# MingXiangL/SPE

Hardware: AMD Instinct MI355X
Metric: images/sec (whole node) at 3x800x1333 bs=2/GPU (higher is better)
Workload: dtype bf16/fp16 operands, fp32 accumulate; 1 GPU; TSCAM_cait_S24 (C=384, depth 24, 8 heads) + 0-layer encoder + 6-layer conditional-DETR decoder x2 stages, 100 queries, COCO heads (91), 2x3x800x1333 per GPU (N=4150 tokens), fwd + SetCriterion + SetCriterionRefine + bwd + grad all-reduce + clip + AdamW; global_batch=2, parallelism=dp1

## Files before the change

spe_amd/csrc/gemm_bf16tn.hip:

```cpp
#include "common.h"

#define GT_BR 64

typedef unsigned int u32x4t_t __attribute__((ext_vector_type(4)));
typedef short s16x4t_t __attribute__((ext_vector_type(4)));
typedef short s16x8t_t __attribute__((ext_vector_type(8)));

struct GemmTNArgs {
    const unsigned short* A; const unsigned short* B; float* C;
    int M, N, R; long lda, ldb, ldc; float alpha;
    int splitk; long slab; int rt_per_split;
};

template <int W>
__device__ __forceinline__ void gt_load(const unsigned short* __restrict__ base, long ld, int r0, int R, int c0, int C, u32x4t_t (&v)[W / 32]) {
    constexpr int CPR = W / 8, RPP = 256 / CPR;
    const int t = threadIdx.x, cc = c0 + (t % CPR) * 8;
    const bool cv = cc < C;
    const int ccl = cv ? cc : 0;
#pragma unroll
    for (int i = 0; i < W / 32; ++i) {
        const int r = r0 + t / CPR + RPP * i;
        const bool ok = cv && r < R;
        const u32x4t_t q = *reinterpret_cast<const u32x4t_t*>(base + (long)min(r, R - 1) * ld + ccl);
        v[i] = ok ? q : (u32x4t_t){0u, 0u, 0u, 0u};
    }
}
template <int W>
__device__ __forceinline__ void gt_stage(unsigned short* lds, const u32x4t_t (&v)[W / 32]) {
    constexpr int CPR = W / 8, RPP = 256 / CPR, LD = W + 8;
    const int t = threadIdx.x;
#pragma unroll
    for (int i = 0; i < W / 32; ++i)
        *reinterpret_cast<u32x4t_t*>(lds + (t / CPR + RPP * i) * LD + (t % CPR) * 8) = v[i];
}
template <int LD>
__device__ __forceinline__ bf16x8_t gt_operand(const unsigned short* tile, int ks, int c0, int lane) {
    typedef __attribute__((address_space(3))) s16x4t_t lds_s4;
    const unsigned short* p = tile + (32 * ks + 8 * (lane >> 4) + ((lane & 15) >> 2)) * LD + c0 + 4 * (lane & 3);
    const s16x4t_t v0 = __builtin_amdgcn_ds_read_tr16_b64_v4i16((lds_s4*)(p));
    const s16x4t_t v1 = __builtin_amdgcn_ds_read_tr16_b64_v4i16((lds_s4*)(p + 4 * LD));
    const s16x8t_t v = __builtin_shufflevector(v0, v1, 0, 1, 2, 3, 4, 5, 6, 7);
    return __builtin_bit_cast(bf16x8_t, v);
}

template <int BM, int BN>
__global__ __launch_bounds__(256) void gemm_bf16tn_kernel(GemmTNArgs p) {
    extern __shared__ __attribute__((aligned(16))) unsigned short smem_tn[];
    constexpr int NFM = BM / 32, NFN = BN / 32, WM = BM / 2, WN = BN / 2;
    constexpr int LDA = BM + 8, LDB = BN + 8;
    constexpr int TA_ = GT_BR * LDA, TB_ = GT_BR * LDB;
    auto sA = [&](int buf) { return smem_tn + buf * (TA_ + TB_); };
    auto sB = [&](int buf) { return smem_tn + buf * (TA_ + TB_) + TA_; };
    const int tiles_m = (p.M + BM - 1) / BM;
    const int tm = blockIdx.x % tiles_m, tn = blockIdx.x / tiles_m;
    const int zs = blockIdx.z;
    float* C = p.C + (long)zs * p.slab;
    const int m0 = tm * BM, n0 = tn * BN;
    const int rtiles = (p.R + GT_BR - 1) / GT_BR;
    const int rt_begin = zs * p.rt_per_split;
    int rt_end = rt_begin + p.rt_per_split; if (rt_end > rtiles) rt_end = rtiles;
    const int nt = rt_end - rt_begin;
    const int lane = threadIdx.x & 63, w = threadIdx.x >> 6;
    const int wm = w >> 1, wn = w & 1, fr = lane & 15;

    f32x4_t acc[NFM][NFN];
#pragma unroll
    for (int i = 0; i < NFM; ++i)
#pragma unroll
        for (int j = 0; j < NFN; ++j) acc[i][j] = (f32x4_t){0.f, 0.f, 0.f, 0.f};

    u32x4t_t ca[BM / 32], cb[BN / 32], na[BM / 32], nb[BN / 32];
#pragma unroll
    for (int i = 0; i < BM / 32; ++i) na[i] = (u32x4t_t){0u, 0u, 0u, 0u};
#pragma unroll
    for (int i = 0; i < BN / 32; ++i) nb[i] = (u32x4t_t){0u, 0u, 0u, 0u};
    if (nt > 0) {
        gt_load<BM>(p.A, p.lda, rt_begin * GT_BR, p.R, m0, p.M, ca);
        gt_load<BN>(p.B, p.ldb, rt_begin * GT_BR, p.R, n0, p.N, cb);
        gt_stage<BM>(sA(0), ca);
        gt_stage<BN>(sB(0), cb);
        if (nt > 1) {
            gt_load<BM>(p.A, p.lda, (rt_begin + 1) * GT_BR, p.R, m0, p.M, ca);
            gt_load<BN>(p.B, p.ldb, (rt_begin + 1) * GT_BR, p.R, n0, p.N, cb);
        }
        __syncthreads();
        for (int t = 0; t < nt; ++t) {
            const int buf = t & 1;
            if (t + 2 < nt) {
                gt_load<BM>(p.A, p.lda, (rt_begin + t + 2) * GT_BR, p.R, m0, p.M, na);
                gt_load<BN>(p.B, p.ldb, (rt_begin + t + 2) * GT_BR, p.R, n0, p.N, nb);
            }
#pragma unroll
            for (int ks = 0; ks < GT_BR / 32; ++ks) {
                bf16x8_t a[NFM], b[NFN];
#pragma unroll
                for (int i = 0; i < NFM; ++i) a[i] = gt_operand<LDA>(sA(buf), ks, wm * WM + i * 16, lane);
#pragma unroll
                for (int j = 0; j < NFN; ++j) b[j] = gt_operand<LDB>(sB(buf), ks, wn * WN + j * 16, lane);
#pragma unroll
                for (int i = 0; i < NFM; ++i)
#pragma unroll
                    for (int j = 0; j < NFN; ++j)
                        acc[i][j] = __builtin_amdgcn_mfma_f32_16x16x32_bf16(b[j], a[i], acc[i][j], 0, 0, 0);
            }
            if (t + 1 < nt) {
                gt_stage<BM>(sA(buf ^ 1), ca);
                gt_stage<BN>(sB(buf ^ 1), cb);
            }
#pragma unroll
            for (int i = 0; i < BM / 32; ++i) ca[i] = na[i];
#pragma unroll
            for (int i = 0; i < BN / 32; ++i) cb[i] = nb[i];
            __syncthreads();
        }
    }
    const bool vst = ((p.ldc & 3) == 0) && ((reinterpret_cast<uintptr_t>(C) & 15) == 0);
#pragma unroll
    for (int j = 0; j < NFN; ++j) {
        const int n = n0 + wn * WN + j * 16 + (lane >> 4) * 4;
        if (n >= p.N) continue;
#pragma unroll
        for (int i = 0; i < NFM; ++i) {
            const int m = m0 + wm * WM + i * 16 + fr;
            if (m >= p.M) continue;
            const long off = (long)m * p.ldc + n;
            float v[4];
#pragma unroll
            for (int r = 0; r < 4; ++r) v[r] = acc[i][j][r] * p.alpha;
            if (vst && n + 3 < p.N) spe_store4_stream(C + off, v[0], v[1], v[2], v[3]);
            else {
#pragma unroll
                for (int r = 0; r < 4; ++r) if (n + r < p.N) C[off + r] = v[r];
            }
        }
    }
}

template <int BM, int BN>
static int launch_tn(const GemmTNArgs& p, hipStream_t stream) {
    constexpr int smem = 2 * GT_BR * ((BM + 8) + (BN + 8)) * (int)sizeof(unsigned short);
    static bool attr_set = false;
    if (!attr_set) {
        hipError_t e = hipFuncSetAttribute(reinterpret_cast<const void*>(&gemm_bf16tn_kernel<BM, BN>),
                                           hipFuncAttributeMaxDynamicSharedMemorySize, smem);
        if (e != hipSuccess) return (int)e;
        attr_set = true;
    }
    const int tiles = ((p.M + BM - 1) / BM) * ((p.N + BN - 1) / BN);
    hipLaunchKernelGGL((gemm_bf16tn_kernel<BM, BN>), dim3(tiles, 1, p.splitk), dim3(256), smem, stream, p);
    SPE_CHECK_LAUNCH();
    return 0;
}

extern "C" int spe_gemm_bf16tn(const void* A16, const void* B16, float* C, int M, int N, int R, long lda, long ldb, long ldc,
                               float alpha, int splitk, hipStream_t stream) {
    if (M <= 0 || N <= 0) return 0;
    if (R <= 0) return -4;
    auto al16 = [](const void* q) { return (reinterpret_cast<uintptr_t>(q) & 15) == 0; };
    if (!al16(A16) || !al16(B16) || (lda & 7) || (ldb & 7) || (M & 7) || (N & 7)) return -2;
    GemmTNArgs p;
    p.A = reinterpret_cast<const unsigned short*>(A16); p.B = reinterpret_cast<const unsigned short*>(B16); p.C = C;
    p.M = M; p.N = N; p.R = R; p.lda = lda; p.ldb = ldb; p.ldc = ldc; p.alpha = alpha; p.slab = 0;
    const int rtiles = (R + GT_BR - 1) / GT_BR;
    if (splitk < 0) { splitk = -splitk; p.slab = (long)M * ldc; if (splitk > rtiles) return -5; }
    else if (splitk > 1) return -2;
    if (splitk < 1) splitk = 1;
    p.splitk = splitk;
    p.rt_per_split = (rtiles + splitk - 1) / splitk;
    const long t128 = (long)((M + 127) / 128) * ((N + 127) / 128) * splitk;
    static const int small_max = SPE_KNOB("SPE_TN_SMALL_TILES", 256);
    if (t128 < small_max) return launch_tn<64, 64>(p, stream);
    if (M > 64 && N > 64) return launch_tn<128, 128>(p, stream);
    if (M > 64) return launch_tn<128, 64>(p, stream);
    return launch_tn<64, 64>(p, stream);
}
```

spe_amd/kernels.py:

```python
import ctypes
import os

import torch

from . import lib

_PRECISION = 2
import functools as _functools
import threading as _threading

_TLS = _threading.local()


def _in_bwd():
    return getattr(_TLS, "in_bwd", False)


def backward_scope(fn):
    @_functools.wraps(fn)
    def wrapped(ctx, *grads):
        prev, _TLS.in_bwd = _in_bwd(), True
        if _DEFER_FLATS is not None and not _FLUSH_QUEUED[0]:
            _FLUSH_QUEUED[0] = True
            try:
                torch.autograd.Variable._execution_engine.queue_callback(_flush_after_backward)
            except RuntimeError:
                _FLUSH_QUEUED[0] = False
        try:
            return fn(ctx, *grads)
        finally:
            _TLS.in_bwd = prev
    return wrapped


_FLUSH_QUEUED = [False]
_DEFER_FLATS = None


def _flush_after_backward():
    _FLUSH_QUEUED[0] = False
    reduce_flush()


def forward_scope(fn):
    @_functools.wraps(fn)
    def wrapped(ctx, *args):
        prev, _TLS.in_bwd = _in_bwd(), False
        try:
            return fn(ctx, *args)
        finally:
            _TLS.in_bwd = prev
    return wrapped


def split_now():
    return _PRECISION == 1 or (_PRECISION == 2 and not _in_bwd())


def split_fwd():
    return _PRECISION == 2 and not _in_bwd()
_RNG = {"seed": None, "offset": 0}


def set_precision(mode):
    global _PRECISION
    _PRECISION = {"bf16": 0, "bf16x3": 1, "bf16s": 2, 0: 0, 1: 1, 2: 2}[mode]


def get_precision():
    return ("bf16", "bf16x3", "bf16s")[_PRECISION]


def manual_seed(seed):
    _RNG["seed"] = int(seed) & 0xFFFFFFFFFFFFFFFF
    _RNG["offset"] = 0


def next_rng():
    if _RNG["seed"] is None:
        _RNG["seed"] = (torch.initial_seed() * 0x9E3779B97F4A7C15 + 0x5EEDC0DE) & 0xFFFFFFFFFFFFFFFF
    _RNG["offset"] += 1
    return _RNG["seed"], _RNG["offset"]


_TIMED = {}


def enable_timing(names):
    _TIMED.clear()
    for n in names:
        _TIMED[n] = []


def timing_results():
    return {n: (len(ev), (sum(a.elapsed_time(b) for a, b in ev) / len(ev)) if ev else 0.0) for n, ev in _TIMED.items()}


_GEMM_DIMS = {"spe_gemm_bf16nt": (7, 8, 9), "spe_gemm_bf16nt_ex": (16, 17, 18)}


_RWS = None
_RWS_BYTES = 16 << 20


_RWS_DEVIDX = -1
_RWS_STREAM = None


def _register_reduce_ws():
    global _RWS
    dev = torch.device("cuda", torch.cuda.current_device())
    _RWS = torch.zeros((_RWS_BYTES,), device=dev, dtype=torch.uint8)
    lib.call("spe_set_reduce_workspace", _RWS.data_ptr(), _RWS_BYTES, _st())


def _guard_reduce_ws(cur, st):
    global _RWS_STREAM, _RWS_DEVIDX
    if _RWS is None:
        _register_reduce_ws()
    if cur != _RWS.device.index:
        raise lib.SpeLibraryError(f"spe_amd kernels were first used on cuda:{_RWS.device.index} and are now launched on cuda:{cur}: "
                                  "the reduction workspace is per process (one process per GPU)")
    if _RWS_STREAM is not None and st != _RWS_STREAM:
        ev = torch.cuda.Event()
        ev.record(torch.cuda.ExternalStream(_RWS_STREAM, device=_RWS.device) if _RWS_STREAM else torch.cuda.default_stream(_RWS.device))
        torch.cuda.current_stream().wait_event(ev)
    _RWS_STREAM, _RWS_DEVIDX = st, cur


DEFER_REDUCE = os.environ.get("SPE_DEFER_REDUCE", "1") != "0"
_DEFER_ARENA = None


def defer_reductions(flats, arena_bytes=48 << 20):
    global _DEFER_ARENA, _DEFER_FLATS
    if _DEFER_FLATS is not None:
        lib.call("spe_reduce_flush", _st())
    if not flats or not DEFER_REDUCE or not flats[0].is_cuda or flats[0].dtype != torch.float32:
        lib.call("spe_reduce_defer_ranges", None, None, 0)
        _DEFER_FLATS = None
        return
    if _DEFER_ARENA is None or _DEFER_ARENA.device != flats[0].device:
        _DEFER_ARENA = torch.empty((arena_bytes,), device=flats[0].device, dtype=torch.uint8)
        lib.call("spe_reduce_defer_arena", _DEFER_ARENA.data_ptr(), arena_bytes)
    n = len(flats)
    ptrs = (ctypes.c_void_p * n)(*[f.data_ptr() for f in flats])
    sizes = (ctypes.c_size_t * n)(*[f.numel() * 4 for f in flats])
    lib.call("spe_reduce_defer_ranges", ptrs, sizes, n)
    _DEFER_FLATS = list(flats)


def reduce_flush():
    if _DEFER_FLATS is not None:
        lib.call("spe_reduce_flush", _st())


def _call(name, *args):
    if _RWS is None:
        _register_reduce_ws()
    if not _TIMED:
        return lib.call(name, *args)
    ev = _TIMED.get(name)
    if ev is None and name in _GEMM_DIMS:
        i, j, k = _GEMM_DIMS[name]
        ev = _TIMED.get("%s:%d,%d,%d" % (name, args[i], args[j], args[k]))
    if ev is None:
        return lib.call(name, *args)
    a, b = torch.cuda.Event(enable_timing=True), torch.cuda.Event(enable_timing=True)
    a.record()
    lib.call(name, *args)
    b.record()
    ev.append((a, b))


_ZPOOL = {"buf": None, "off": 0}
_ZPOOL_FLOATS = 4 << 20


def zeros_small(n, device):
    if n > (1 << 18):
        return torch.zeros((n,), device=device, dtype=torch.float32)
    na = (n + 63) & ~63
    z = _ZPOOL
    if z["buf"] is None or z["buf"].device != device or z["off"] + na > z["buf"].numel():
        z["buf"] = torch.zeros((_ZPOOL_FLOATS,), device=device, dtype=torch.float32)
        z["off"] = 0
    out = z["buf"][z["off"]:z["off"] + n]
    z["off"] += na
    return out


def grad_buffer(param):
    if param is None or not getattr(param, "_spe_grad_fresh", False) or getattr(param, "_spe_shared", False):
        return None
    param._spe_grad_fresh = False
    param._spe_handed = True
    buf = param._spe_grad_buf
    return buf.view_as(buf)


ACC_ZERO_MAX = 16384


def _zeros_or(buf, n, device):
    if buf is None:
        return zeros_small(n, device)
    v = buf.view(-1)
    if v.numel() > ACC_ZERO_MAX:
        v.zero_()
    return v


def _p(t):
    return None if t is None else t.data_ptr()


_raw_stream = getattr(torch._C, "_cuda_getCurrentRawStream", None)


def _st():
    cur = torch.cuda.current_device()
    st = _raw_stream(cur) if _raw_stream is not None else torch.cuda.current_stream().cuda_stream
    if st != _RWS_STREAM or cur != _RWS_DEVIDX:
        _guard_reduce_ws(cur, st)
    return st


def _chk(*ts):
    for t in ts:
        if t is None:
            continue
        if not t.is_cuda:
            raise lib.SpeLibraryError("spe_amd kernels run on the GPU only (got a CPU tensor); there is no CPU fallback")
        if t.dtype != torch.float32:
            raise TypeError(f"expected float32, got {t.dtype}")


TN_SMALL_MAX = 256


def auto_splitk(M, N, K, batch):
    tiles = ((M + 127) // 128) * ((N + 127) // 128) * batch
    if tiles >= 256 or K < 1024:
        return 1
    sk = max(1, min(512 // tiles, K // 512, 16))
    if batch == 1 and tiles * sk < TN_SMALL_MAX:
        t64 = ((M + 63) // 64) * ((N + 63) // 64)
        sk = max(1, min(512 // t64, K // 512, 16))
    return sk


def gemm(A, B, C, M, N, K, lda, ldb, ldc, transA=False, transB=False, bias=None, C2=None,
         batch0=1, batch1=1, sA=(0, 0), sB=(0, 0), sC=(0, 0), alpha=1.0, act=0, splitk=1):
    _call("spe_gemm_f32", _p(A), _p(B), _p(C), _p(bias), _p(C2), M, N, K, lda, ldb, ldc,
             int(transA), int(transB), batch0, batch1, sA[0], sA[1], sB[0], sB[1], sC[0], sC[1],
             float(alpha), int(act), int(splitk), int(split_now()), _st())
    return C


LINEAR16 = True
LINEAR16_MIN_ROWS = 128
_W16 = {}
_W16_EPOCH = 0


def weights_changed():
    global _W16_EPOCH
    _W16_EPOCH += 1


LINEAR_SMALL_MAX_ROWS = 2048


def _lin_small_ok(R, N, K):
    return LINEAR16 and _PRECISION != 1 and LINEAR16_MIN_ROWS <= R < LINEAR_SMALL_MAX_ROWS and N % 8 == 0 and K % 8 == 0


def _lin16_ok(R, N, K):
    return LINEAR16 and _PRECISION != 1 and R >= LINEAR16_MIN_ROWS and N % 8 == 0 and K % 8 == 0


def cvt_bf16(x2, want=True, wantT=False, ldt=None, colsum_out=None, act_aux=None, act=0, out=None, ldo=None, out_lo=None, lo_f16=False):
    _chk(x2)
    R, C = x2.shape
    if out is None:
        out = torch.empty((R, C), device=x2.device, dtype=torch.bfloat16) if want else None
        ldo = C
    outT = None
    if wantT:
        ldt = ldt or ((R + 63) // 64) * 64
        outT = torch.empty((C, ldt), device=x2.device, dtype=torch.bfloat16)
    if lo_f16:
        assert colsum_out is None and act_aux is None and out_lo is not None and out_lo.dtype == torch.float16
        _call("spe_cvt_bf16_h", _p(x2), x2.stride(0), R, C, _p(out), _p(out_lo), ldo or C, _p(outT), ldt or 0, _st())
        return out, outT
    _call("spe_cvt_bf16", _p(x2), x2.stride(0), R, C, _p(out), _p(out_lo), ldo or C, _p(outT), ldt or 0, _p(colsum_out), _p(act_aux),
          int(act), _st())
    return out, outT


_W16_TABLE = None
_W16_REFRESHED = -1


def _refresh_weights16():
    global _W16_TABLE, _W16_REFRESHED
    import numpy as np
    live = []
    for key, ent in list(_W16.items()):
        owner = ent[0]()
        if owner is None or not _owns(owner, key[0]):
            del _W16[key]
            continue
        live.append((key, owner, ent))
    _W16_REFRESHED = _W16_EPOCH
    if not live:
        return
    sig = tuple((k, e[3].data_ptr(), e[4].data_ptr(), e[5].data_ptr() if e[5] is not None else 0, e[5].dtype if e[5] is not None else None)
                for k, _, e in live)
    if _W16_TABLE is None or _W16_TABLE[0] != sig:
        rec = np.zeros(len(live), dtype=np.dtype([("x", "<u8"), ("out", "<u8"), ("outT", "<u8"), ("ldt", "<i8"), ("R", "<i4"),
                                                   ("C", "<i4"), ("tile0", "<i4"), ("tiles_c", "<i4"), ("out_lo", "<u8"), ("flags", "<i8")]))
        t0 = 0
        for i, ((ptr, R, C), _, e) in enumerate(live):
            tc = (C + 63) // 64
            rec[i] = (ptr, e[3].data_ptr(), e[4].data_ptr(), e[4].shape[1], R, C, t0, tc, e[5].data_ptr() if e[5] is not None else 0,
                      1 if (e[5] is not None and e[5].dtype == torch.float16) else 0)
            t0 += tc * ((max(R, e[4].shape[1]) + 63) // 64)
        table = host_table(rec.view(np.uint8), live[0][2][3].device)
        _W16_TABLE = (sig, table, len(live), t0)
    _, table, n, tiles = _W16_TABLE
    _call("spe_cvt_bf16_multi", _p(table), n, tiles, _st())
    for key, owner, e in live:
        _W16[key] = (e[0], owner._version, _W16_EPOCH, e[3], e[4], e[5])


def _owns(owner, ptr):
    base = owner.data_ptr()
    return base <= ptr < base + max(1, owner.numel()) * owner.element_size()


def host_table(bytes_np, device):
    pin = torch.from_numpy(bytes_np.copy()).pin_memory()
    dev = torch.empty(pin.shape, dtype=torch.uint8, device=device)
    dev.copy_(pin, non_blocking=True)
    dev._spe_pin = pin
    return dev


def weight16(W, lo=False, f16=False):
    import weakref
    key = (W.data_ptr(), W.shape[0], W.shape[1])
    ent = _W16.get(key)
    if ent is not None:
        owner = ent[0]()
        if owner is not None and _owns(owner, key[0]):
            if ent[2] != _W16_EPOCH and _W16_REFRESHED != _W16_EPOCH:
                _refresh_weights16()
                ent = _W16.get(key, ent)
            if ent[1] == owner._version and ent[2] == _W16_EPOCH and (not lo or (ent[5] is not None and (ent[5].dtype == torch.float16) == f16)):
                return (ent[3], ent[4], ent[5]) if lo else (ent[3], ent[4])
            if not lo and ent[5] is not None and ent[5].dtype == torch.float16:
                f16 = True
    owner = W._base if W._base is not None else W
    want_lo = lo or f16 or _PRECISION == 2
    with torch.no_grad():
        W16lo = torch.empty(W.shape, device=W.device, dtype=torch.float16 if f16 else torch.bfloat16) if want_lo else None
        W16, W16T = cvt_bf16(W.detach(), True, True, ldt=W.shape[0], out_lo=W16lo, lo_f16=f16)
    if len(_W16) > 4096:
        _W16.clear()
    _W16[key] = (weakref.ref(owner), owner._version, _W16_EPOCH, W16, W16T, W16lo)
    return (W16, W16T, W16lo) if lo else (W16, W16T)


_WCAT = {}


def weightcat16(Ws, bs, lo=False):
    import weakref
    key = tuple((W.data_ptr(), tuple(W.shape)) for W in Ws)
    vers = tuple(W._version for W in Ws) + tuple(b._version for b in bs)
    ent = _WCAT.get(key)
    if ent is not None and ent[1] == _W16_EPOCH and ent[2] == vers and (ent[6] is not None or not lo):
        owners = [r() for r in ent[0]]
        if all(o is not None and _owns(o, W.data_ptr()) for o, W in zip(owners, Ws)) and ent[3].shape == (sum(W.shape[0] for W in Ws), Ws[0].shape[1]):
            return (ent[3], ent[4], ent[5], ent[6]) if lo else (ent[3], ent[4], ent[5])
    with torch.no_grad():
        trip = [weight16(W, lo=lo) for W in Ws]
        Wc = torch.cat([t_[0] for t_ in trip], 0)
        WcT = torch.cat([t_[1] for t_ in trip], 1)
        Wclo = torch.cat([t_[2] for t_ in trip], 0) if lo else None
        bc = torch.cat([b.detach() for b in bs])
    if len(_WCAT) > 64:
        _WCAT.clear()
    _WCAT[key] = ([weakref.ref(W._base if W._base is not None else W) for W in Ws], _W16_EPOCH, vers, Wc, WcT, bc, Wclo)
    return (Wc, WcT, bc, Wclo) if lo else (Wc, WcT, bc)


def gemm_splitk_into(A, B, out, M, N, K, lda, ldb, ldc, transA, transB, batch0, batch1, sA, sB, sC, alpha=1.0):
    sk = auto_splitk(M, N, K, batch0 * batch1)
    if sk <= 1:
        return gemm(A, B, out, M, N, K, lda, ldb, ldc, transA, transB, batch0=batch0, batch1=batch1, sA=sA, sB=sB, sC=sC, alpha=alpha)
    extent = (((batch0 - 1) * sC[0] + (batch1 - 1) * sC[1] + (M - 1) * ldc + N) + 3) & ~3
    assert out.is_contiguous() and extent <= out.numel() + 3
    ws = torch.empty((sk, extent), device=out.device, dtype=torch.float32)
    gemm(A, B, ws, M, N, K, lda, ldb, ldc, transA, transB, batch0=batch0, batch1=batch1, sA=sA, sB=sB, sC=sC, alpha=alpha, splitk=-sk)
    out.zero_()
    n = out.numel()
    _call("spe_colsum", _p(ws), _p(out), sk, n, extent, 1, _st())
    return out


def gemm16(A16, B16, C, M, N, K, lda, ldb, ldc, bias=None, C2=None, alpha=1.0, act=0, splitk=1, Alo=None, Blo=None):
    _call("spe_gemm_bf16nt", _p(A16), _p(B16), _p(Alo), _p(Blo), _p(C), _p(bias), _p(C2), M, N, K, lda, ldb, ldc, float(alpha), int(act),
          int(splitk), _st())
    return C


def cvt_f16(x2, out=None):
    R, C = x2.shape
    if out is None:
        out = torch.empty((R, C), device=x2.device, dtype=torch.float16)
    _call("spe_cvt_f16", _p(x2), x2.stride(0), R, C, _p(out), out.stride(0), _st())
    return out


_WCATH = {}


def weightcat_f16(Ws, bs):
    import weakref
    key = tuple((W.data_ptr(), tuple(W.shape)) for W in Ws)
    vers = tuple(W._version for W in Ws) + tuple(b._version for b in bs)
    ent = _WCATH.get(key)
    if ent is not None and ent[1] == _W16_EPOCH and ent[2] == vers:
        owners = [r() for r in ent[0]]
        if all(o is not None and _owns(o, W.data_ptr()) for o, W in zip(owners, Ws)):
            return ent[3], ent[4]
    with torch.no_grad():
        Wh = cvt_f16(torch.cat([W.detach() for W in Ws], 0))
        bc = torch.cat([b.detach() for b in bs])
    if len(_WCATH) > 64:
        _WCATH.clear()
    _WCATH[key] = ([weakref.ref(W._base if W._base is not None else W) for W in Ws], _W16_EPOCH, vers, Wh, bc)
    return Wh, bc


def kv_frags(ym16, yp16, L, B, S, H, dh, train):
    dev = ym16.device
    nt, dk = (S + 15) // 16, 2 * dh
    Kf = torch.empty((L, B, H, nt, (dk + 31) // 32, 64, 8), device=dev, dtype=torch.float16)
    V16 = torch.empty((L, B, H, nt, (dh + 15) // 16, 64, 4), device=dev, dtype=torch.float16)
    K16 = torch.empty((L, B, H, nt, (dk + 15) // 16, 64, 4), device=dev, dtype=torch.bfloat16) if train else None
    Vf = torch.empty((L, B, H, nt, (dh + 31) // 32, 64, 8), device=dev, dtype=torch.bfloat16) if train else None
    _call("spe_kv_frags", _p(ym16), ym16.stride(0), _p(yp16), yp16.stride(0), _p(Kf), _p(V16), _p(K16), _p(Vf), L, B, S, H, dh, _st())
    return Kf, V16, K16, Vf


def kv_grad_scatter(dk, dv, dYm, dYp, layer, B, S, H, dh):
    _call("spe_kv_grad_scatter", _p(dk), _p(dv), _p(dYm), dYm.stride(0), _p(dYp), dYp.stride(0), int(layer), B, S, H, dh, _st())


def colsum_bf16_blocks(x16, blkC, outs):
    n = len(outs)
    ptrs = (ctypes.c_void_p * n)(*[o.data_ptr() for o in outs])
    _call("spe_colsum_bf16_blocks", _p(x16), x16.stride(0), x16.shape[0], n, int(blkC), ptrs, 0, _st())


def gemm16_tn(A16, B16, C, M, N, R, lda, ldb, ldc, alpha=1.0, splitk=1):
    _call("spe_gemm_bf16tn", _p(A16), _p(B16), _p(C), M, N, R, lda, ldb, ldc, float(alpha), int(splitk), _st())
    return C


def gemm16_ex(A16, B16, M, N, K, lda, ldb, bias=None, C=None, C2=None, out16=None, out16T=None, colsum=None, aux=None,
              alpha=1.0, act=0, res=None, rgamma=None, Alo=None, Blo=None, out16lo=None, drop=None, sscale=None, rps=1, op_f16=False):
    half_flags = (1 if (C2 is not None and C2.dtype == torch.float16) else 0) | (2 if (aux is not None and aux.dtype == torch.float16) else 0)
    if op_f16:
        assert A16.dtype == torch.float16 and B16.dtype == torch.float16 and Alo is None and Blo is None
        half_flags |= 4 | (8 if out16lo is not None else 0)
        assert out16lo is None or out16lo.dtype == torch.float16
    if (drop is not None and drop[0] > 0) or sscale is not None:
        pd, sd, of = drop if (drop is not None and drop[0] > 0) else (0.0, 0, 0)
        _call("spe_gemm_bf16nt_exd", _p(A16), _p(B16), _p(Alo), _p(Blo), _p(C), _p(bias), _p(C2), _p(out16), _p(out16lo), N, _p(out16T),
              out16T.shape[1] if out16T is not None else 0, _p(colsum), _p(aux), _p(res), _p(rgamma), M, N, K, lda, ldb, N,
              float(alpha), int(act), half_flags, float(pd), int(sd), int(of), _p(sscale), int(rps), _st())
        return
    _call("spe_gemm_bf16nt_ex", _p(A16), _p(B16), _p(Alo), _p(Blo), _p(C), _p(bias), _p(C2), _p(out16), _p(out16lo), N, _p(out16T),
          out16T.shape[1] if out16T is not None else 0, _p(colsum), _p(aux), _p(res), _p(rgamma), M, N, K, lda, ldb, N,
          float(alpha), int(act), half_flags, _st())


def mlp16_ok(R, K, Hd, N):
    return _lin16_ok(R, Hd, K) and _lin16_ok(R, N, Hd)




def layerscale_residual_bwd16(dout2, y2, gamma, Rp, db_out=None, dg_out=None, want_rowmajor=True, want_T=True, drop=None, sscale=None, rps=1):
    R, C = dout2.shape
    dev = dout2.device
    dy16 = torch.empty((R, C), device=dev, dtype=torch.bfloat16) if want_rowmajor else None
    dy16T = torch.empty((C, Rp), device=dev, dtype=torch.bfloat16) if want_T else None
    db = _zeros_or(db_out, C, dev)
    dg = _zeros_or(dg_out, C, dev)
    if (drop is not None and drop[0] > 0) or sscale is not None:
        pd, sd, of = drop if (drop is not None and drop[0] > 0) else (0.0, 0, 0)
        _call("spe_layerscale_residual_bwd16d", _p(dout2), _p(y2), int(y2.dtype == torch.float16), _p(gamma), _p(dy16), _p(dy16T), Rp, _p(db),
              _p(dg), R, C, float(pd), int(sd), int(of), _p(sscale), int(rps), _st())
        return dy16, dy16T, db, dg
    _call("spe_layerscale_residual_bwd16", _p(dout2), _p(y2), int(y2.dtype == torch.float16), _p(gamma), _p(dy16), _p(dy16T), Rp, _p(db), _p(dg),
          R, C, _st())
    return dy16, dy16T, db, dg


def linear_res_fwd(x2, W, b, res, gamma, save=True, src=None, drop=None, sscale=None, rps=1):
    R, K = x2.shape
    N = W.shape[0]
    dev = x2.device
    sp = split_fwd()
    x16, x16lo = act16(x2, src, want_lo=sp)
    out = torch.empty((R, N), device=dev, dtype=torch.float32)
    y = torch.empty((R, N), device=dev, dtype=torch.float16 if MLP_PRE_F16 else torch.float32) if save else None
    Wt = weight16(W, lo=sp)
    gemm16_ex(x16, Wt[0], R, N, K, K, K, bias=b, C=out, C2=y, res=res, rgamma=gamma, Alo=x16lo, Blo=Wt[2] if sp else None,
              drop=drop, sscale=sscale, rps=rps)
    return out, (x16, y)


def linear_res_bwd(dout2, saved, W, gamma, need_dx=True, grad_bufs=(None, None, None), drop=None, sscale=None, rps=1, pre=None):
    x16, y = saved
    R, N = dout2.shape
    K = W.shape[1]
    gW, gb, gg = grad_bufs
    if pre is not None:
        dy16, db, dg = pre
    else:
        dy16, _, db, dg = layerscale_residual_bwd16(dout2, y, gamma, ((R + 63) // 64) * 64, db_out=gb, dg_out=gg, want_rowmajor=True, want_T=False,
                                                    drop=drop, sscale=sscale, rps=rps)
    dW = _dw16_tn(dy16, x16, N, K, R, gW)
    dx = None
    if need_dx:
        dx = torch.empty((R, K), device=dout2.device, dtype=torch.float32)
        gemm16(dy16, weight16(W)[1], dx, R, K, N, N, N, K)
    return dx, dW, db, dg


MLP_PRE_F16 = False


MLP_F16 = True


def mlp_f16_ok(R, K, Hd, N):
    return (MLP_F16 and split_fwd() and R >= 2048 and K % 64 == 0 and K >= 128 and Hd % 64 == 0 and Hd >= 128 and N % 8 == 0 and N >= 64)


def mlp_gelu_fwd(x2, W1, b1, W2, b2, res=None, gamma=None, save=True, src=None, drop1=None, drop2=None, sscale=None, rps=1):
    R, K = x2.shape
    Hd, N = W1.shape[0], W2.shape[0]
    dev = x2.device
    sp = split_fwd()
    if res is not None and mlp_f16_ok(R, K, Hd, N):
        x16, xh = act16(x2, src, want_lo=True, lo_f16=True)
        pre = torch.empty((R, Hd), device=dev, dtype=torch.float16 if MLP_PRE_F16 else torch.float32) if save else None
        h16 = torch.empty((R, Hd), device=dev, dtype=torch.bfloat16)
        hh = torch.empty((R, Hd), device=dev, dtype=torch.float16)
        W1h, W2h = weight16(W1, lo=True, f16=True)[2], weight16(W2, lo=True, f16=True)[2]
        gemm16_ex(xh, W1h, R, Hd, K, K, K, bias=b1, C2=pre, out16=h16, act=2, out16lo=hh, drop=drop1, op_f16=True)
        out = torch.empty((R, N), device=dev, dtype=torch.float32)
        y = torch.empty((R, N), device=dev, dtype=torch.float16 if MLP_PRE_F16 else torch.float32) if save else None
        gemm16_ex(hh, W2h, R, N, Hd, Hd, Hd, bias=b2, C=out, C2=y, res=res, rgamma=gamma, drop=drop2, sscale=sscale, rps=rps, op_f16=True)
        return out, (x16, pre, h16, y)
    x16, x16lo = act16(x2, src, want_lo=sp)
    pre = torch.empty((R, Hd), device=dev, dtype=torch.float16 if MLP_PRE_F16 else torch.float32) if save else None
    h16 = torch.empty((R, Hd), device=dev, dtype=torch.bfloat16)
    h16lo = torch.empty((R, Hd), device=dev, dtype=torch.bfloat16) if sp else None
    W1t, W2t = weight16(W1, lo=sp), weight16(W2, lo=sp)
    W1lo, W2lo = (W1t[2], W2t[2]) if sp else (None, None)
    gemm16_ex(x16, W1t[0], R, Hd, K, K, K, bias=b1, C2=pre, out16=h16, act=2, Alo=x16lo, Blo=W1lo, out16lo=h16lo, drop=drop1)
    y = torch.empty((R, N), device=dev, dtype=torch.float32)
    if res is None:
        gemm16(h16, W2t[0], y, R, N, Hd, Hd, Hd, N, bias=b2, Alo=h16lo, Blo=W2lo)
        return y, (x16, pre, h16)
    out = torch.empty((R, N), device=dev, dtype=torch.float32)
    if MLP_PRE_F16:
        y = torch.empty((R, N), device=dev, dtype=torch.float16)
    gemm16_ex(h16, W2t[0], R, N, Hd, Hd, Hd, bias=b2, C=out, C2=y if save else None, res=res, rgamma=gamma, Alo=h16lo, Blo=W2lo,
              drop=drop2, sscale=sscale, rps=rps)
    return out, (x16, pre, h16, y)


def _dw_slabs(launch, sk, N, K, dW_out, dev):
    if sk > 1:
        ws = torch.empty((sk, N * K), device=dev, dtype=torch.float32)
        launch(ws, -sk)
        return colsum(ws, out=None if dW_out is None else dW_out.view(-1), accumulate=dW_out is None).view(N, K)
    dW = dW_out if dW_out is not None else torch.empty((N, K), device=dev, dtype=torch.float32)
    launch(dW, 1)
    return dW


def _dw16_tn(dy16, x16, N, K, R, dW_out, lda=None):
    lda = N if lda is None else lda
    sk = min(auto_splitk(N, K, R, 1), max(1, R // 64))
    return _dw_slabs(lambda C, splitk: gemm16_tn(dy16, x16, C, N, K, R, lda, K, K, splitk=splitk), sk, N, K, dW_out, dy16.device)


def mlp_gelu_bwd(dy2, saved, W1, W2, need_dx=True, grad_bufs=(None, None, None, None), gamma=None, dg_out=None,
                 drop1=None, drop2=None, sscale=None, rps=1, ls_pre=None):
    x16, pre, h16 = saved[:3]
    R, N = dy2.shape
    Hd, K = W1.shape
    dev = dy2.device
    gW1, gb1, gW2, gb2 = grad_bufs
    dg = None
    if ls_pre is not None and gamma is None:
        raise RuntimeError("spe_amd.kernels.mlp_gelu_bwd: a LayerNorm backward took this node's LayerScale part, but the node cannot consume it")
    if ls_pre is not None:
        dy16, db2, dg = ls_pre
    elif gamma is not None:
        dy16, _, db2, dg = layerscale_residual_bwd16(dy2, saved[3], gamma, ((R + 63) // 64) * 64, db_out=gb2, dg_out=dg_out, want_T=False,
                                                     drop=drop2, sscale=sscale, rps=rps)
    else:
        db2 = _zeros_or(gb2, N, dev)
        dy16, _ = cvt_bf16(dy2, True, False, colsum_out=db2)
    dW2 = _dw16_tn(dy16, h16, N, Hd, R, gW2)
    db1 = _zeros_or(gb1, Hd, dev)
    dp16 = torch.empty((R, Hd), device=dev, dtype=torch.bfloat16)
    gemm16_ex(dy16, weight16(W2)[1], R, Hd, N, N, N, out16=dp16, colsum=db1, aux=pre, act=2, drop=drop1)
    dW1 = _dw16_tn(dp16, x16, Hd, K, R, gW1)
    dx = None
    if need_dx:
        dx = torch.empty((R, K), device=dev, dtype=torch.float32)
        gemm16(dp16, weight16(W1)[1], dx, R, K, Hd, Hd, Hd, K)
    if gamma is not None:
        return dx, dW1, db1, dW2, db2, dg
    return dx, dW1, db1, dW2, db2


def act16(x2, src=None, want_lo=False, lo_f16=False):
    if src is not None:
        ent = getattr(src, "_spe16", None)
        if (ent is not None and ent[0] == src._version and ent[1].shape == x2.shape
                and (not want_lo or (ent[3] is not None and (ent[3].dtype == torch.float16) == lo_f16))):
            return ent[1], (ent[3] if want_lo else None)
    x16lo = torch.empty(x2.shape, device=x2.device, dtype=torch.float16 if lo_f16 else torch.bfloat16) if want_lo else None
    x16, _ = cvt_bf16(x2, True, False, out_lo=x16lo, lo_f16=lo_f16 and want_lo)
    if src is not None:
        attach16(src, x16, x16lo)
    return x16, x16lo


def linear_fwd(x2, W, b, act=0, want_pre=False, save_for_dw=True, src=None):
    _chk(x2, W, b)
    R, K = x2.shape
    N = W.shape[0]
    y = torch.empty((R, N), device=x2.device, dtype=torch.float32)
    pre = torch.empty_like(y) if want_pre else None
    if _lin_small_ok(R, N, K) and W.is_contiguous():
        sp = split_fwd()
        Wt = weight16(W, lo=sp)
        ent = getattr(src, "_spe16", None) if src is not None else None
        x16 = ent[1] if (ent is not None and ent[0] == src._version and ent[1].shape == x2.shape) else None
        x16_out = None
        if x16 is None and save_for_dw:
            x16 = x16_out = torch.empty((R, K), device=x2.device, dtype=torch.bfloat16)
            if src is not None:
                attach16(src, x16)
        _call("spe_linear_small_fwd", _p(x2), x2.stride(0), _p(Wt[0]), _p(Wt[2] if sp else None), _p(b), _p(y), _p(pre), _p(x16_out),
              R, N, K, N, int(act), _st())
        return y, pre, (x16 if save_for_dw else x2)
    if _lin16_ok(R, N, K) and W.is_contiguous():
        sp = split_fwd()
        x16, x16lo = act16(x2, src, want_lo=sp)
        Wt = weight16(W, lo=sp)
        gemm16(x16, Wt[0], y, R, N, K, K, K, N, bias=b, C2=pre, act=act, Alo=x16lo, Blo=Wt[2] if sp else None)
        return y, pre, (x16 if save_for_dw else x2)
    gemm(x2, W, y, R, N, K, K, K, N, False, True, bias=b, C2=pre, act=act)
    return y, pre, x2


def linear_group_ok(R, Ws, bs):
    N, K = Ws[0].shape
    return (2 <= len(Ws) <= 16 and _lin_small_ok(R, N, K) and N % 128 == 0
            and all(W.shape == Ws[0].shape and W.is_contiguous() for W in Ws) and all(b is not None for b in bs))


def _ptr_array(ptrs):
    return (ctypes.c_void_p * len(ptrs))(*[(p if p else None) for p in ptrs])


def linear_group_fwd(x2, Ws, bs, src=None, adds=None):
    _chk(x2, *Ws)
    R, K = x2.shape
    N = Ws[0].shape[0]
    sp = split_fwd()
    trip = [weight16(W, lo=sp) for W in Ws]
    ent = getattr(src, "_spe16", None) if src is not None else None
    x16 = ent[1] if (ent is not None and ent[0] == src._version and ent[1].shape == x2.shape) else None
    x16_out = None
    if x16 is None:
        x16 = x16_out = torch.empty((R, K), device=x2.device, dtype=torch.bfloat16)
        if src is not None:
            attach16(src, x16)
    ys = [torch.empty((R, N), device=x2.device, dtype=torch.float32) for _ in Ws]
    _call("spe_linear_small_group_fwd", _p(x2), x2.stride(0), _ptr_array([t_[0].data_ptr() for t_ in trip]),
          _ptr_array([t_[2].data_ptr() for t_ in trip]) if sp else None, _ptr_array([b.data_ptr() for b in bs]),
          _ptr_array([0 if a is None else a.data_ptr() for a in adds]) if adds is not None else None,
          _ptr_array([y.data_ptr() for y in ys]), _p(x16_out), R, len(Ws), N, K, _st())
    return ys, x16


def linear_group_bwd(dys, x16, Ws, need_dx, dW_outs, db_outs):
    n = len(Ws)
    N, K = Ws[0].shape
    R = x16.shape[0]
    dev = x16.device
    dx = torch.empty((R, K), device=dev, dtype=torch.float32) if need_dx else None
    dWs, dbs = [], []
    for i in range(n):
        if dys[i] is None:
            dWs.append(None); dbs.append(None)
            continue
        dWs.append(dW_outs[i] if dW_outs[i] is not None else torch.empty((N, K), device=dev, dtype=torch.float32))
        dbs.append(db_outs[i].view(-1) if db_outs[i] is not None else torch.empty((N,), device=dev, dtype=torch.float32))
    _call("spe_linear_small_group_bwd", _ptr_array([0 if d is None else d.data_ptr() for d in dys]), _p(x16),
          _ptr_array([weight16(W)[1].data_ptr() for W in Ws]) if need_dx else None, _p(dx),
          _ptr_array([0 if w is None else w.data_ptr() for w in dWs]), _ptr_array([0 if b is None else b.data_ptr() for b in dbs]),
          R, n, N, K, _st())
    return dx, dWs, dbs


def linear_bwd(dy2, xsave, W, need_dx=True, need_dw=True, need_db=True, dW_out=None, db_out=None, act=0, act_aux=None):
    _chk(dy2, W)
    R, N = dy2.shape
    K = W.shape[1]
    dx = dW = db = None
    x16 = xsave.dtype == torch.bfloat16
    if (x16 or not need_dw) and _lin_small_ok(R, N, K) and W.is_contiguous():
        dev = dy2.device
        if need_dx:
            dx = torch.empty((R, K), device=dev, dtype=torch.float32)
        if need_dw:
            dW = dW_out if dW_out is not None else torch.empty((N, K), device=dev, dtype=torch.float32)
        if need_db:
            db = db_out.view(-1) if db_out is not None else torch.empty((N,), device=dev, dtype=torch.float32)
        _call("spe_linear_small_bwd", _p(dy2), _p(act_aux if act else None), int(act), _p(xsave if need_dw else None),
              _p(weight16(W)[1] if need_dx else None), _p(dx), _p(dW), _p(db), R, N, K, _st())
        return dx, dW, db
    if (x16 or not need_dw) and _lin16_ok(R, N, K) and W.is_contiguous():
        if need_db:
            db = _zeros_or(db_out, N, dy2.device)
        dy16, _ = cvt_bf16(dy2, need_dx or need_dw, False, colsum_out=db, act_aux=act_aux if act else None, act=act)
        need_db = False
        if need_dx:
            dx = torch.empty((R, K), device=dy2.device, dtype=torch.float32)
            gemm16(dy16, weight16(W)[1], dx, R, K, N, N, N, K)
        if need_dw:
            dW = _dw16_tn(dy16, xsave, N, K, R, dW_out)
    else:
        if x16:
            raise RuntimeError("linear_bwd: bf16 activations were saved but the bf16 GEMM path is disabled now")
        if act:
            dy2 = act_bwd(dy2, act_aux, act)
        x2 = xsave
        if need_dx:
            dx = torch.empty((R, K), device=dy2.device, dtype=torch.float32)
            gemm(dy2, W, dx, R, K, N, N, K, K, False, False)
        if need_dw:
            dW = _dw_slabs(lambda C, splitk: gemm(dy2, x2, C, N, K, R, N, K, K, True, False, splitk=splitk), auto_splitk(N, K, R, 1), N, K,
                           dW_out, dy2.device)
    if need_db:
        db = _zeros_or(db_out, N, dy2.device)
        _call("spe_colsum", _p(dy2), _p(db), R, N, N, 1, _st())
    return dx, dW, db


def colsum(x2, out=None, accumulate=True):
    _chk(x2)
    R, C = x2.shape
    if out is None:
        out = zeros_small(C, x2.device)
    _call("spe_colsum", _p(x2), _p(out), R, C, x2.stride(0), int(bool(accumulate)), _st())
    return out


def act_bwd(dy, aux, mode):
    _chk(dy, aux)
    dx = torch.empty_like(dy)
    _call("spe_act_bwd", _p(dy), _p(aux), _p(dx), dy.numel(), mode, _st())
    return dx


def layernorm_fwd(x2, g, b, eps, want16=False, f16=False):
    _chk(x2, g, b)
    R, C = x2.shape
    y = torch.empty_like(x2)
    mean = torch.empty((R,), device=x2.device, dtype=torch.float32)
    rstd = torch.empty_like(mean)
    y16 = torch.empty((R, C), device=x2.device, dtype=torch.bfloat16) if want16 else None
    f16 = f16 and want16 and split_fwd()
    y16lo = torch.empty((R, C), device=x2.device, dtype=torch.float16 if f16 else torch.bfloat16) if (want16 and split_fwd()) else None
    _call("spe_layernorm_fwd_h" if f16 else "spe_layernorm_fwd", _p(x2), _p(g), _p(b), _p(y), _p(mean), _p(rstd), R, C, float(eps), _p(y16), _p(y16lo), _st())
    return (y, mean, rstd, y16, y16lo) if want16 else (y, mean, rstd)


def produces16(R, C):
    return LINEAR16 and _PRECISION != 1 and R >= LINEAR16_MIN_ROWS and C % 8 == 0


def attach16(t, x16, x16lo=None):
    t._spe16 = (t._version, x16, None, x16lo)


LN_LS_FUSE = True


def layernorm_bwd(dy2, x2, g, mean, rstd, dg_out=None, db_out=None, add=None, ls=None):
    _chk(dy2, x2, g)
    R, C = x2.shape
    dx = torch.empty_like(x2)
    dg = _zeros_or(dg_out, C, x2.device)
    db = _zeros_or(db_out, C, x2.device)
    if ls is not None:
        y, lgam, ls_db_out, ls_dg_out = ls
        dy16 = torch.empty((R, C), device=x2.device, dtype=torch.bfloat16)
        ldb = _zeros_or(ls_db_out, C, x2.device)
        ldg = _zeros_or(ls_dg_out, C, x2.device)
        _call("spe_layernorm_bwd_ls", _p(dy2), _p(x2), _p(g), _p(mean), _p(rstd), _p(dx), _p(dg), _p(db), R, C, _p(add), _p(y), _p(lgam), _p(dy16),
              _p(ldb), _p(ldg), _st())
        return dx, dg, db, (dy16, ldb, ldg)
    _call("spe_layernorm_bwd", _p(dy2), _p(x2), _p(g), _p(mean), _p(rstd), _p(dx), _p(dg), _p(db), R, C, _p(add), _st())
    return dx, dg, db


def layernorm_res_fwd(x2, z2, g, b, eps, p, seed, offset):
    _chk(x2, z2, g, b)
    R, C = x2.shape
    y, sm = torch.empty_like(x2), torch.empty_like(x2)
    mean = torch.empty((R,), device=x2.device, dtype=torch.float32)
    rstd = torch.empty_like(mean)
    _call("spe_layernorm_res_fwd", _p(x2), _p(z2), _p(g), _p(b), _p(sm), _p(y), _p(mean), _p(rstd), R, C, float(eps), float(p), seed,
          offset, _st())
    return y, sm, mean, rstd


def layernorm_res_bwd(dy2, sm, g, mean, rstd, p, seed, offset, dg_out=None, db_out=None, dy_b=None):
    R, C = sm.shape
    ds = torch.empty_like(sm)
    dz = torch.empty_like(sm) if p > 0 else None
    dg = _zeros_or(dg_out, C, sm.device)
    db = _zeros_or(db_out, C, sm.device)
    _call("spe_layernorm_res_bwd", _p(dy2), _p(dy_b), _p(sm), _p(g), _p(mean), _p(rstd), _p(ds), _p(dz), _p(dg), _p(db), R, C, float(p), seed,
          offset, _st())
    return ds, (dz if dz is not None else ds), dg, db


def layerscale_residual_fwd(x2, y2, gamma, sample_scale, rows_per_sample):
    _chk(x2, y2, gamma, sample_scale)
    R, C = x2.shape
    out = torch.empty_like(x2)
    _call("spe_layerscale_residual_fwd", _p(x2), _p(y2), _p(gamma), _p(sample_scale), _p(out), R, C,
             rows_per_sample, _st())
    return out


def layerscale_residual_bwd(dout2, y2, gamma, sample_scale, rows_per_sample, dg_out=None):
    _chk(dout2, y2, gamma, sample_scale)
    R, C = dout2.shape
    dy = torch.empty_like(dout2)
    dg = _zeros_or(dg_out, C, dout2.device)
    _call("spe_layerscale_residual_bwd", _p(dout2), _p(y2), _p(gamma), _p(sample_scale), _p(dy), _p(dg), R, C,
             rows_per_sample, _st())
    return dy, dg


def dropout(x, p, seed, offset):
    _chk(x)
    y = torch.empty_like(x)
    _call("spe_dropout", _p(x), _p(y), x.numel(), float(p), seed, offset, _st())
    return y


def pad4(n):
    return (n + 3) // 4 * 4


def softmax_fwd(S, mask_u8, B, H, Nq, Nk, ld, p_drop, seed, offset):
    Pd = torch.empty_like(S) if p_drop > 0 else None
    _call("spe_softmax_fwd", _p(S), _p(mask_u8), _p(S), _p(Pd), B, H, Nq, Nk, ld, float(p_drop), seed, offset, _st())
    return S, Pd


def softmax_bwd(dPd, P, B, H, Nq, Nk, ld, p_drop, seed, offset):
    _call("spe_softmax_bwd", _p(dPd), _p(P), _p(dPd), B, H, Nq, Nk, ld, float(p_drop), seed, offset, _st())
    return dPd


def talking_fwd(S, Wl, bl, Ww, bw, B, H, Nq, Nk, ld, p_drop, seed, offset):
    Pd = torch.empty_like(S)
    _call("spe_talking_softmax_fwd", _p(S), _p(Wl), _p(bl), _p(Ww), _p(bw), _p(S), _p(Pd), B, H, Nq, Nk, ld,
             float(p_drop), seed, offset, _st())
    return S, Pd


def talking_bwd(dPd, P, S, Wl, Ww, B, H, Nq, Nk, ld, p_drop, seed, offset):
    nblocks = min(B * Nq, 1024)
# ... 470 lines not shown
```

Baseline: 42.26 images/sec.

## Stream TN weight-gradient GEMM tiles directly into swizzled LDS with multi-stage pipeline

Replaces the register-staged double buffer in the bf16 TN GEMM (used for weight gradients) with direct global-to-LDS loads via global_load_lds_dwordx4. Operand tiles go into an XOR-swizzled unpadded layout, with a 2- or 3-stage ring gated by vmcnt waits. The kernel also requests two workgroups per CU. It remaps a flattened grid so that groups of 8 split-K slices of one tile launch adjacently, and adds a split-K heuristic preferring 8 or 16 splits. The aim is to cut register pressure and LDS store cost and to improve load overlap and L2 locality. The risks are inline asm m0 handling, zero-filling of the tail, and correctness of the swizzle.

```diff
diff --git a/spe_amd/csrc/gemm_bf16tn.hip b/spe_amd/csrc/gemm_bf16tn.hip
--- a/spe_amd/csrc/gemm_bf16tn.hip
+++ b/spe_amd/csrc/gemm_bf16tn.hip
@@ -9,52 +9,58 @@
 struct GemmTNArgs {
     const unsigned short* A; const unsigned short* B; float* C;
     int M, N, R; long lda, ldb, ldc; float alpha;
-    int splitk; long slab; int rt_per_split;
+    int splitk; long slab; int rt_per_split; int bind;
 };
 
+__device__ __forceinline__ void gt_glds16(const void* gsrc, unsigned lds_dst) {
+    unsigned keep;
+    asm volatile("s_mov_b32 %0, m0\n\ts_mov_b32 m0, %2\n\ts_nop 0\n\tglobal_load_lds_dwordx4 %1, off\n\ts_mov_b32 m0, %0"
+                 : "=&s"(keep) : "v"(gsrc), "s"(lds_dst) : "memory");
+}
+
 template <int W>
-__device__ __forceinline__ void gt_load(const unsigned short* __restrict__ base, long ld, int r0, int R, int c0, int C, u32x4t_t (&v)[W / 32]) {
-    constexpr int CPR = W / 8, RPP = 256 / CPR;
-    const int t = threadIdx.x, cc = c0 + (t % CPR) * 8;
-    const bool cv = cc < C;
-    const int ccl = cv ? cc : 0;
+__device__ __forceinline__ int gt_slot(int r, int gc) {
+    if constexpr (W == 128) return gc ^ (((r & 3) | (((r >> 3) & 1) << 2)) << 1);
+    else return gc ^ ((((r >> 1) & 1) | (((r >> 3) & 1) << 1)) << 1);
+}
+
+template <int W>
+__device__ __forceinline__ void gt_issue(const unsigned short* __restrict__ base, long ld, int r0, int R, int c0, int C, unsigned lds, int ws, int lane) {
+    constexpr int CPR = W / 8;
+    static_assert((GT_BR * W) % 2048 == 0 && (W == 64 || W == 128), "whole pieces per wave");
 #pragma unroll
-    for (int i = 0; i < W / 32; ++i) {
-        const int r = r0 + t / CPR + RPP * i;
-        const bool ok = cv && r < R;
-        const u32x4t_t q = *reinterpret_cast<const u32x4t_t*>(base + (long)min(r, R - 1) * ld + ccl);
-        v[i] = ok ? q : (u32x4t_t){0u, 0u, 0u, 0u};
+    for (int i = 0; i < GT_BR * W / 2048; ++i) {
+        const int c = 64 * (i * 4 + ws) + lane, row = c / CPR;
+        const int cc = c0 + gt_slot<W>(row, c % CPR) * 8;
+        const int r = min(r0 + row, R - 1);
+        gt_glds16(base + (long)r * ld + (cc < C ? cc : 0), lds + (unsigned)((i * 4 + ws) * 1024));
     }
 }
 template <int W>
-__device__ __forceinline__ void gt_stage(unsigned short* lds, const u32x4t_t (&v)[W / 32]) {
-    constexpr int CPR = W / 8, RPP = 256 / CPR, LD = W + 8;
-    const int t = threadIdx.x;
-#pragma unroll
-    for (int i = 0; i < W / 32; ++i)
-        *reinterpret_cast<u32x4t_t*>(lds + (t / CPR + RPP * i) * LD + (t % CPR) * 8) = v[i];
-}
-template <int LD>
 __device__ __forceinline__ bf16x8_t gt_operand(const unsigned short* tile, int ks, int c0, int lane) {
     typedef __attribute__((address_space(3))) s16x4t_t lds_s4;
-    const unsigned short* p = tile + (32 * ks + 8 * (lane >> 4) + ((lane & 15) >> 2)) * LD + c0 + 4 * (lane & 3);
+    const int row = 32 * ks + 8 * (lane >> 4) + ((lane & 15) >> 2);
+    const unsigned short* p = tile + row * W + gt_slot<W>(row, c0 >> 3) * 8 + 4 * (lane & 3);
     const s16x4t_t v0 = __builtin_amdgcn_ds_read_tr16_b64_v4i16((lds_s4*)(p));
-    const s16x4t_t v1 = __builtin_amdgcn_ds_read_tr16_b64_v4i16((lds_s4*)(p + 4 * LD));
+    const s16x4t_t v1 = __builtin_amdgcn_ds_read_tr16_b64_v4i16((lds_s4*)(p + 4 * W));
     const s16x8t_t v = __builtin_shufflevector(v0, v1, 0, 1, 2, 3, 4, 5, 6, 7);
     return __builtin_bit_cast(bf16x8_t, v);
 }
 
 template <int BM, int BN>
-__global__ __launch_bounds__(256) void gemm_bf16tn_kernel(GemmTNArgs p) {
+__global__ __launch_bounds__(256, 2) void gemm_bf16tn_kernel(GemmTNArgs p) {
     extern __shared__ __attribute__((aligned(16))) unsigned short smem_tn[];
     constexpr int NFM = BM / 32, NFN = BN / 32, WM = BM / 2, WN = BN / 2;
-    constexpr int LDA = BM + 8, LDB = BN + 8;
-    constexpr int TA_ = GT_BR * LDA, TB_ = GT_BR * LDB;
-    auto sA = [&](int buf) { return smem_tn + buf * (TA_ + TB_); };
-    auto sB = [&](int buf) { return smem_tn + buf * (TA_ + TB_) + TA_; };
-    const int tiles_m = (p.M + BM - 1) / BM;
-    const int tm = blockIdx.x % tiles_m, tn = blockIdx.x / tiles_m;
-    const int zs = blockIdx.z;
+    constexpr int NST = (BM + BN > 192) ? 2 : 3;
+    constexpr int TA_ = GT_BR * BM, STE = GT_BR * (BM + BN);
+    constexpr int PW = GT_BR * (BM + BN) / 2048;
+    const int tiles_m = (p.M + BM - 1) / BM, tiles = tiles_m * ((p.N + BN - 1) / BN);
+    int tile, zs;
+    if (p.bind) {
+        const int idx = blockIdx.x >> 3;
+        zs = (blockIdx.x & 7) + 8 * (idx / tiles); tile = idx % tiles;
+    } else { tile = blockIdx.x % tiles; zs = blockIdx.x / tiles; }
+    const int tm = tile % tiles_m, tn = tile / tiles_m;
     float* C = p.C + (long)zs * p.slab;
     const int m0 = tm * BM, n0 = tn * BN;
     const int rtiles = (p.R + GT_BR - 1) / GT_BR;
@@ -62,7 +68,9 @@
     int rt_end = rt_begin + p.rt_per_split; if (rt_end > rtiles) rt_end = rtiles;
     const int nt = rt_end - rt_begin;
     const int lane = threadIdx.x & 63, w = threadIdx.x >> 6;
+    const int ws = __builtin_amdgcn_readfirstlane(w);
     const int wm = w >> 1, wn = w & 1, fr = lane & 15;
+    const unsigned lds0 = __builtin_amdgcn_readfirstlane((unsigned)(uintptr_t)(__attribute__((address_space(3))) unsigned short*)smem_tn);
 
     f32x4_t acc[NFM][NFN];
 #pragma unroll
@@ -70,49 +78,42 @@
 #pragma unroll
         for (int j = 0; j < NFN; ++j) acc[i][j] = (f32x4_t){0.f, 0.f, 0.f, 0.f};
 
-    u32x4t_t ca[BM / 32], cb[BN / 32], na[BM / 32], nb[BN / 32];
+    auto issue = [&](int t) {
+        const unsigned dst = lds0 + (unsigned)((t % NST) * STE * 2);
+        const int r0 = (rt_begin + t) * GT_BR;
+        gt_issue<BM>(p.A, p.lda, r0, p.R, m0, p.M, dst, ws, lane);
+        gt_issue<BN>(p.B, p.ldb, r0, p.R, n0, p.N, dst + TA_ * 2, ws, lane);
+    };
 #pragma unroll
-    for (int i = 0; i < BM / 32; ++i) na[i] = (u32x4t_t){0u, 0u, 0u, 0u};
+    for (int st = 0; st < NST - 1; ++st) if (st < nt) issue(st);
+    for (int t = 0; t < nt; ++t) {
+        if (t + NST - 1 <= nt) asm volatile("s_waitcnt vmcnt(%0)" :: "n"((NST - 2) * PW) : "memory");
+        else asm volatile("s_waitcnt vmcnt(0)" ::: "memory");
+        __builtin_amdgcn_s_barrier();
+        asm volatile("" ::: "memory");
+        if (t + NST - 1 < nt) issue(t + NST - 1);
+        unsigned short* sA = smem_tn + (t % NST) * STE;
+        unsigned short* sB = sA + TA_;
+        const int rem = p.R - (rt_begin + t) * GT_BR;
+        if (rem < GT_BR) {
+            for (int c = rem * (BM / 8) + (int)threadIdx.x; c < GT_BR * (BM / 8); c += 256)
+                *reinterpret_cast<u32x4t_t*>(sA + c * 8) = (u32x4t_t){0u, 0u, 0u, 0u};
+            for (int c = rem * (BN / 8) + (int)threadIdx.x; c < GT_BR * (BN / 8); c += 256)
+                *reinterpret_cast<u32x4t_t*>(sB + c * 8) = (u32x4t_t){0u, 0u, 0u, 0u};
+            __syncthreads();
+        }
 #pragma unroll
-    for (int i = 0; i < BN / 32; ++i) nb[i] = (u32x4t_t){0u, 0u, 0u, 0u};
-    if (nt > 0) {
-        gt_load<BM>(p.A, p.lda, rt_begin * GT_BR, p.R, m0, p.M, ca);
-        gt_load<BN>(p.B, p.ldb, rt_begin * GT_BR, p.R, n0, p.N, cb);
-        gt_stage<BM>(sA(0), ca);
-        gt_stage<BN>(sB(0), cb);
-        if (nt > 1) {
-            gt_load<BM>(p.A, p.lda, (rt_begin + 1) * GT_BR, p.R, m0, p.M, ca);
-            gt_load<BN>(p.B, p.ldb, (rt_begin + 1) * GT_BR, p.R, n0, p.N, cb);
-        }
-        __syncthreads();
-        for (int t = 0; t < nt; ++t) {
-            const int buf = t & 1;
-            if (t + 2 < nt) {
-                gt_load<BM>(p.A, p.lda, (rt_begin + t + 2) * GT_BR, p.R, m0, p.M, na);
-                gt_load<BN>(p.B, p.ldb, (rt_begin + t + 2) * GT_BR, p.R, n0, p.N, nb);
-            }
+        for (int ks = 0; ks < GT_BR / 32; ++ks) {
+            bf16x8_t a[NFM], b[NFN];
 #pragma unroll
-            for (int ks = 0; ks < GT_BR / 32; ++ks) {
-                bf16x8_t a[NFM], b[NFN];
+            for (int i = 0; i < NFM; ++i) a[i] = gt_operand<BM>(sA, ks, wm * WM + i * 16, lane);
 #pragma unroll
-                for (int i = 0; i < NFM; ++i) a[i] = gt_operand<LDA>(sA(buf), ks, wm * WM + i * 16, lane);
+            for (int j = 0; j < NFN; ++j) b[j] = gt_operand<BN>(sB, ks, wn * WN + j * 16, lane);
 #pragma unroll
-                for (int j = 0; j < NFN; ++j) b[j] = gt_operand<LDB>(sB(buf), ks, wn * WN + j * 16, lane);
+            for (int i = 0; i < NFM; ++i)
 #pragma unroll
-                for (int i = 0; i < NFM; ++i)
-#pragma unroll
-                    for (int j = 0; j < NFN; ++j)
-                        acc[i][j] = __builtin_amdgcn_mfma_f32_16x16x32_bf16(b[j], a[i], acc[i][j], 0, 0, 0);
-            }
-            if (t + 1 < nt) {
-                gt_stage<BM>(sA(buf ^ 1), ca);
-                gt_stage<BN>(sB(buf ^ 1), cb);
-            }
-#pragma unroll
-            for (int i = 0; i < BM / 32; ++i) ca[i] = na[i];
-#pragma unroll
-            for (int i = 0; i < BN / 32; ++i) cb[i] = nb[i];
-            __syncthreads();
+                for (int j = 0; j < NFN; ++j)
+                    acc[i][j] = __builtin_amdgcn_mfma_f32_16x16x32_bf16(b[j], a[i], acc[i][j], 0, 0, 0);
         }
     }
     const bool vst = ((p.ldc & 3) == 0) && ((reinterpret_cast<uintptr_t>(C) & 15) == 0);
@@ -138,8 +139,8 @@
 }
 
 template <int BM, int BN>
-static int launch_tn(const GemmTNArgs& p, hipStream_t stream) {
-    constexpr int smem = 2 * GT_BR * ((BM + 8) + (BN + 8)) * (int)sizeof(unsigned short);
+static int launch_tn(GemmTNArgs p, hipStream_t stream) {
+    constexpr int smem = ((BM + BN > 192) ? 2 : 3) * GT_BR * (BM + BN) * (int)sizeof(unsigned short);
     static bool attr_set = false;
     if (!attr_set) {
         hipError_t e = hipFuncSetAttribute(reinterpret_cast<const void*>(&gemm_bf16tn_kernel<BM, BN>),
@@ -148,7 +149,9 @@
         attr_set = true;
     }
     const int tiles = ((p.M + BM - 1) / BM) * ((p.N + BN - 1) / BN);
-    hipLaunchKernelGGL((gemm_bf16tn_kernel<BM, BN>), dim3(tiles, 1, p.splitk), dim3(256), smem, stream, p);
+    p.bind = (p.splitk % 8 == 0) ? 1 : 0;
+    const int grid = tiles * p.splitk;
+    hipLaunchKernelGGL((gemm_bf16tn_kernel<BM, BN>), dim3(grid), dim3(256), smem, stream, p);
     SPE_CHECK_LAUNCH();
     return 0;
 }
@@ -161,7 +164,7 @@
     if (!al16(A16) || !al16(B16) || (lda & 7) || (ldb & 7) || (M & 7) || (N & 7)) return -2;
     GemmTNArgs p;
     p.A = reinterpret_cast<const unsigned short*>(A16); p.B = reinterpret_cast<const unsigned short*>(B16); p.C = C;
-    p.M = M; p.N = N; p.R = R; p.lda = lda; p.ldb = ldb; p.ldc = ldc; p.alpha = alpha; p.slab = 0;
+    p.M = M; p.N = N; p.R = R; p.lda = lda; p.ldb = ldb; p.ldc = ldc; p.alpha = alpha; p.slab = 0; p.bind = 0;
     const int rtiles = (R + GT_BR - 1) / GT_BR;
     if (splitk < 0) { splitk = -splitk; p.slab = (long)M * ldc; if (splitk > rtiles) return -5; }
     else if (splitk > 1) return -2;
diff --git a/spe_amd/kernels.py b/spe_amd/kernels.py
--- a/spe_amd/kernels.py
+++ b/spe_amd/kernels.py
@@ -248,6 +248,19 @@
         t64 = ((M + 63) // 64) * ((N + 63) // 64)
         sk = max(1, min(512 // t64, K // 512, 16))
     return sk
+
+
+def tn_splitk(M, N, R):
+    t128 = ((M + 127) // 128) * ((N + 127) // 128)
+    t64 = ((M + 63) // 64) * ((N + 63) // 64)
+    if t128 < 256:
+        for sk in (8, 16):
+            if sk > R // 512:
+                break
+            wgs = (t64 if t128 * sk < TN_SMALL_MAX else t128) * sk
+            if TN_SMALL_MAX <= wgs <= 512:
+                return sk
+    return auto_splitk(M, N, R, 1)
 
 
 def gemm(A, B, C, M, N, K, lda, ldb, ldc, transA=False, transB=False, bias=None, C2=None,
@@ -602,7 +615,7 @@
 
 def _dw16_tn(dy16, x16, N, K, R, dW_out, lda=None):
     lda = N if lda is None else lda
-    sk = min(auto_splitk(N, K, R, 1), max(1, R // 64))
+    sk = min(tn_splitk(N, K, R), max(1, R // 64))
     return _dw_slabs(lambda C, splitk: gemm16_tn(dy16, x16, C, N, K, R, lda, K, K, splitk=splitk), sk, N, K, dW_out, dy16.device)
 
 
```

Result: no change. 42.04 images/sec (-0.5%).
